# andr345/frtm-vos

Measured on AMD Instinct MI355X. Metric: segmented frames/sec/GPU (480p, ResNet101, full CG iters), higher is better.
Workload: dtype f32

## Files before the change

### frtm-vos_amd/_hip.py

```python
import ctypes
import os

import torch

_HERE = os.path.dirname(os.path.abspath(__file__))
LIB_PATH = os.path.join(_HERE, 'libfrtm_hip.so')

P, I, F, D = ctypes.c_void_p, ctypes.c_int, ctypes.c_float, ctypes.c_double


class ConvDesc(ctypes.Structure):
    _fields_ = [(k, I) for k in ('B', 'Cin', 'Hin', 'Win', 'Cout', 'ksize', 'stride', 'pad',
                                 'relu', 'out_transposed', 'splitk', 'tile', 'w_layout', 'ws_elems', 'w_pitch')]


SIGNATURES = {
    'frtm_last_error': (ctypes.c_char_p, []),
    'frtm_version': (I, []),
    'frtm_device_info': (I, [P]),
    'frtm_pixel_weights': (I, [P, I, I, I, I, F, P, P, P]),
    'frtm_normal_build': (I, [P, I, P, I, I, I, I, I, F, P, I, P, P, P, P, P]),
    'frtm_memory_next_slot': (I, [P, I, F, I, P, P, I, P]),
    'frtm_memory_insert': (I, [P, P, I, P, P]),
    'frtm_filter_scores': (I, [P, P, I, I, I, I, P, I, P]),
# ... 51 lines not shown
    'frtm_conv_persistent_launches': (ctypes.c_long, []),
    'frtm_conv_last_kernels': (ctypes.c_char_p, []),
    'frtm_conv_bf16x3_launches': (ctypes.c_long, []),
    'frtm_conv_bf16x1_launches': (ctypes.c_long, []),
    'frtm_conv_bf16x1_3x3_launches': (ctypes.c_long, []),
    'frtm_conv_bf16x1_3x3s2_launches': (ctypes.c_long, []),
    'frtm_telea_inpaint_u8': (I, [P, P, I, I, I, I, P]),
    'frtm_fastdiv_check': (ctypes.c_uint, [ctypes.c_uint, ctypes.c_uint]),
    'frtm_backbone_set_lanes': (I, [P, I]),
    'frtm_backbone_generation': (I, [P]),
    'frtm_backbone_set_winograd': (I, [P, I]),
    'frtm_backbone_set_winograd4': (I, [P, I]),
    'frtm_backbone_set_precision': (I, [P, I]),
    'frtm_backbone_set_bf16_pieces': (I, [P, I]),
    'frtm_backbone_set_bf16x1_3x3': (I, [P, I]),
    'frtm_merge_masks': (I, [P, I, I, P]),
    'frtm_merge_masks_frames': (I, [P, I, I, I, P]),
    'frtm_count_above': (I, [P, I, I, F, P, P]),
    'frtm_track_merge': (I, [P, I, I, I, P, P, P, I, P, F, P]),
    'frtm_filter_scores_pitched': (I, [P, P, I, I, I, I, P, I, I, P]),
    'frtm_bilinear_resize': (I, [P, I, I, I, P, I, I, P]),
    'frtm_tse_inject': (I, [P, P, P, P, I, I, I, I, I, I, I, P, P]),
    'frtm_cab_combine': (I, [P, P, P, I, I, I, I, I, I, I, P, P]),
    'frtm_pyrup2x': (I, [P, I, I, I, P, P]),
    'frtm_plane_mean': (I, [P, I, I, P, P]),
    'frtm_conv_wgrad_ws_elems': (ctypes.c_size_t, [I, I, I, I, I, I]),
    'frtm_conv_wgrad': (I, [P, P, I, I, I, I, I, I, P, P, P, ctypes.c_size_t, P]),
    'frtm_conv_wgrad_bf16x1_ws_elems': (ctypes.c_size_t, [I, I, I, I, I]),
    'frtm_conv_wgrad_bf16x1': (I, [P, P, I, I, I, I, I, P, P, P, ctypes.c_size_t, P]),
    'frtm_conv_wgrad_bf16x1_launches': (ctypes.c_long, []),
# ... 271 lines not shown
```

### frtm-vos_amd/build.py

```python
import os
import subprocess
import sys

HERE = os.path.dirname(os.path.abspath(__file__))
CSRC = os.path.join(HERE, 'csrc')
LIB = os.path.join(HERE, 'libfrtm_hip.so')
SOURCES = ['target_model.hip', 'target_apply_grouped.hip', 'cg_persistent.hip', 'joint_persistent.hip', 'joint_fit.hip', 'wide_maps.hip', 'conv_igemm.hip', 'conv_gemm32.hip', 'conv_wino.hip', 'conv_wino4.hip', 'conv_bf16x3.hip', 'conv_bf16x1.hip', 'conv3x3_bf16x1.hip', 'conv3x3s2_bf16x1.hip', 'conv_wgrad_bf16x1.hip', 'backbone.hip', 'image_ops.hip', 'refiner_ops.hip', 'refiner_train.hip', 'telea_host.hip', 'jf_eval.hip', 'train_step.hip', 'frame_resize.hip']
HIPCC = os.environ.get('HIPCC', '/opt/rocm/bin/hipcc')
FLAGS = ['--offload-arch=gfx950', '-O3', '-std=c++17', '-fPIC', '-Wall', '-Wno-unused-function']
if os.environ.get('FRTM_BUILD_ABLATE'):
    FLAGS.append('-DFRTM_DEBUG_ABLATE')


def _stale(target, deps):
    if not os.path.exists(target):
        return True
    t = os.path.getmtime(target)
    return any(os.path.getmtime(d) > t for d in deps)


def build(force=False, verbose=True):
    headers = [os.path.join(CSRC, 'frtm_common.h'), os.path.join(CSRC, 'conv_common.h'), os.path.join(CSRC, 'resident_grid.h'), os.path.join(CSRC, 'resample_taps.h'), os.path.join(os.path.dirname(HERE), 'include', 'frtm_hip.h'), __file__]
    objs = []
    for src in SOURCES:
        sp = os.path.join(CSRC, src)
        if not os.path.exists(sp):
            continue
        obj = os.path.join(CSRC, src.replace('.hip', '.o'))
        objs.append(obj)
        if force or _stale(obj, [sp] + headers):
            cmd = [HIPCC] + FLAGS + ['-c', sp, '-o', obj]
            if verbose:
                print(' '.join(cmd), flush=True)
            subprocess.check_call(cmd)
    if force or _stale(LIB, objs):
        cmd = [HIPCC, '--offload-arch=gfx950', '-shared', '-fPIC'] + objs + ['-o', LIB]
        if verbose:
# ... 8 lines not shown
```

### frtm-vos_amd/csrc/backbone.hip

```cpp
#include <vector>
#include <algorithm>
#include <mutex>
#include <chrono>
#include <cstdio>
#include "frtm_common.h"
#include "../../include/frtm_hip.h"

void frtm_conv_plan(int M, int Ntot, int nchunks, int vec1x1, int* tile, int* splitk);

struct ConvL {
  int Cout, Cin, ks, stride, pad;
  float* wT = nullptr; float* scale = nullptr; float* shift = nullptr; int* ktab = nullptr;
  float* wW = nullptr;
  float* wW4 = nullptr;
  float* wW6 = nullptr;
  float* wB = nullptr;
  float* wB1 = nullptr;
  float* wB3 = nullptr;
  bool loaded = false;
  int layout = 0;
  int plan_tile = 0, plan_splitk = 0;
};
struct BlockL { int conv[3]; int nconv; int ds; };

// ... 11 lines not shown
  bool bottleneck = false;
  std::vector<ConvL> convs;
  std::vector<std::vector<BlockL>> stages;
  std::vector<Lane> lanes = std::vector<Lane>(1);
  int nlanes = 1;
  hipEvent_t fork = nullptr, fork1 = nullptr;
  double last_flops = 0.0;
  double last_flops_form[4] = {0.0, 0.0, 0.0, 0.0};
  double last_flops_exec = 0.0;
  int last_launches = 0;
  bool use_winograd = true;
  int use_winograd4 = getenv("FRTM_NO_WINO4") ? 0 : getenv("FRTM_NO_WINO6") ? 1 : 2;
  int wino4_min_tiles = getenv("FRTM_WINO4_MIN_TILES") ? atoi(getenv("FRTM_WINO4_MIN_TILES")) : 256;
  int precision = 0;
  int bf16x1_min_cols = getenv("FRTM_BF16X1_MIN_COLS") ? atoi(getenv("FRTM_BF16X1_MIN_COLS")) : -1;
  bool bf16x1_3x3 = false;
  int generation = 0;
};

__global__ __launch_bounds__(256) void k_normalize_u8(const unsigned char* __restrict__ img, int H, int W, int P, const float* __restrict__ sc,
                                                       const float* __restrict__ bi, float* __restrict__ out, int planes) {
  const int Wp = W + 2 * P, Hp = H + 2 * P, q4 = (Wp + 3) / 4;
  const size_t total = (size_t)planes * Hp * q4;
  for (size_t i = (size_t)blockIdx.x * 256 + threadIdx.x; i < total; i += (size_t)gridDim.x * 256) {
    const int xq = (int)(i % q4);
    const size_t r = i / q4;
    const int yp = (int)(r % Hp), pl = (int)(r / Hp), c = pl % 3;
    const int y = yp - P;
    const float s = sc[c], b = bi[c];
    float* o = out + ((size_t)pl * Hp + yp) * Wp + xq * 4;
    const unsigned char* src = img + ((size_t)pl * H + (y < 0 || y >= H ? 0 : y)) * W;
#pragma unroll
    for (int j = 0; j < 4; ++j) {
      const int xp = xq * 4 + j, x = xp - P;
      if (xp < Wp) o[j] = (y >= 0 && y < H && x >= 0 && x < W) ? s * (float)src[x] + b : 0.f;
    }
  }
}

typedef float f32x2u __attribute__((ext_vector_type(2), aligned(4)));
__global__ __launch_bounds__(256) void k_maxpool3s2(const float* __restrict__ in, int Hin, int Win, int Ho, int Wo, float* __restrict__ out) {
  const int ox = blockIdx.x * 64 + threadIdx.x, oy = blockIdx.y * 4 + threadIdx.y;
  if (ox >= Wo || oy >= Ho) return;
  const float* ip = in + (size_t)blockIdx.z * Hin * Win;
  const int x0 = ox * 2;
  const bool left = x0 >= 1, pair = x0 + 1 < Win;
  float m = -INFINITY;
#pragma unroll
  for (int dy = 0; dy < 3; ++dy) {
    const int yy = oy * 2 - 1 + dy;
    if ((unsigned)yy >= (unsigned)Hin) continue;
    const float* row = ip + (size_t)yy * Win + x0;
// ... 145 lines not shown
  if (!c.wB3) FRTM_HIP(hipMalloc((void**)&c.wB3, FRTM_CONV_BF16X1_3X3_ELEMS(c.Cout, c.Cin) * sizeof(float)));
  const int layout = c.stride == 2 ? FRTM_WLAYOUT_BF16X1_3X3_S2 : FRTM_WLAYOUT_BF16X1_3X3;
  if (w_oihw) return frtm_conv_pack_weights(w_oihw, c.Cout, c.Cin, 3, layout, c.wB3, nullptr, (frtm_stream_t)st);
  float* tmp = nullptr;
  const size_t total = (size_t)c.Cout * c.Cin * 9;
  FRTM_HIP(hipMalloc((void**)&tmp, total * sizeof(float)));
  k_halo_to_oihw<<<(int)std::min<size_t>((total + 255) / 256, 2048), 256, 0, st>>>(c.wT, c.Cout, c.Cin, (c.Cout + 31) / 32 * 32, tmp);
  int rc = FRTM_ERR_HIP;
  if (hipGetLastError() == hipSuccess) rc = frtm_conv_pack_weights(tmp, c.Cout, c.Cin, 3, layout, c.wB3, nullptr, (frtm_stream_t)st);
  else frtm_set_error("backbone: k_halo_to_oihw failed to launch");
  (void)hipStreamSynchronize(st);
  (void)hipFree(tmp);
  return rc;
}

static int run_conv(frtm_backbone* bb, Lane& ln, int idx, int B, int Hin, int Win, const float* in, const float* residual, int relu,
                    float* out, int* Ho, int* Wo, hipStream_t st, int pad_override = -1) {
  ConvL& c = bb->convs[idx];
  if (!c.loaded) { frtm_set_error("backbone: conv %d has no weights (call frtm_backbone_set_conv)", idx); return FRTM_ERR_STATE; }
  const int pad = pad_override >= 0 ? pad_override : c.pad;
  frtm_conv_desc d;
  d.B = B; d.Cin = c.Cin; d.Hin = Hin; d.Win = Win; d.Cout = c.Cout; d.ksize = c.ks; d.stride = c.stride; d.pad = pad;
  d.relu = relu; d.out_transposed = 0; d.splitk = 0; d.tile = 0; d.w_pitch = 0; d.w_layout = c.layout; d.ws_elems = 0;
  *Ho = (Hin + 2 * pad - c.ks) / c.stride + 1;
  *Wo = (Win + 2 * pad - c.ks) / c.stride + 1;
  {
    const size_t out_elems = (size_t)c.Cout * B * (*Ho) * (*Wo);
    const size_t w = std::min((size_t)FRTM_CONV_MAX_SPLITK * out_elems, (size_t)16 * 1024 * 1024);
    int rc = ensure(bb, &ln.ws, &ln.ws_elems, std::max(w, out_elems * 2));
    if (rc) return rc;
  }
  d.ws_elems = (int)std::min<size_t>(ln.ws_elems, 0x7fffffff);
  bb->last_launches += 1;
  bb->last_flops += 2.0 * c.Cout * (double)B * (*Ho) * (*Wo) * c.Cin * c.ks * c.ks;
  if (bb->precision == 2 && bb->bf16x1_3x3 && c.wB3 && pad == 1 && !c.plan_tile && !c.plan_splitk && bf16x1_3x3_route(bb, c, B, *Ho, *Wo)) {
    d.w_layout = c.stride == 2 ? FRTM_WLAYOUT_BF16X1_3X3_S2 : FRTM_WLAYOUT_BF16X1_3X3;
    d.splitk = 1;
    bb->last_flops_exec += 2.0 * c.Cout * (double)B * (*Ho) * (*Wo) * c.Cin * 9.0;
    bb->last_flops_form[0] += 2.0 * c.Cout * (double)B * (*Ho) * (*Wo) * c.Cin * 9.0;
    return frtm_conv2d(&d, in, c.wB3, nullptr, c.scale, c.shift, residual, out, nullptr, st);
  }
  if (c.wW4 && bb->use_winograd && bb->use_winograd4) {
    int best_m = 0; long best_cost = 0, best_T = 0, best_Tp = 0;
    for (int m : {6, 4}) {
      if (m == 6 && (bb->use_winograd4 < 2 || !c.wW6)) continue;
      const int th = ceil_div(*Ho, m), tw = ceil_div(*Wo, m), NP = (m + 2) * (m + 2);
      const long T = (long)B * th * tw, Tp = (T + 63) / 64 * 64;
      if ((long)ceil_div(c.Cout, 64) * (NP * Tp / 64) < bb->wino4_min_tiles || (long)m * m * th * tw * 4 > (long)5 * (*Ho) * (*Wo) ||
          (size_t)NP * std::max(c.Cin, c.Cout) * Tp * 4 >= 0x7fffffffull)
        continue;
      if (!best_m || NP * Tp < best_cost) { best_m = m; best_cost = NP * Tp; best_T = T; best_Tp = Tp; }
    }
    if (best_m) {
      const int NP = (best_m + 2) * (best_m + 2);
      const size_t need = (size_t)NP * (c.Cin + c.Cout) * best_Tp;
      int rc = ensure(bb, &ln.ws4, &ln.ws4_elems, need);
// ... 41 lines not shown
__global__ void k_clock_probe(long long ticks, unsigned long long* out2) {
  const long long t0 = wall_clock64();
  const unsigned long long c0 = __builtin_readcyclecounter();
  long long t1 = t0;
  for (int it = 0; it < (1 << 22) && (t1 = wall_clock64()) - t0 < ticks; ++it) __builtin_amdgcn_s_sleep(32);
  out2[0] = __builtin_readcyclecounter() - c0;
  out2[1] = (unsigned long long)(t1 - t0);
}

static size_t arena_elems_per_image(const frtm_backbone* bb, int H, int W) {
  const int Hs = (H + 6 - 7) / 2 + 1, Ws = (W + 6 - 7) / 2 + 1;
  size_t need = (size_t)64 * Hs * Ws;
  int ah = (Hs + 1) / 2, aw = (Ws + 1) / 2;
  const int exp = bb->bottleneck ? 4 : 1;
  for (int s = 0; s < 4; ++s) {
    if (s > 0) { ah = (ah + 1) / 2; aw = (aw + 1) / 2; }
    need = std::max(need, (size_t)(64 << s) * exp * ah * aw);
    need = std::max(need, (size_t)(64 << s) * (s > 0 ? 4 : 1) * ah * aw);
  }
  const int P = bb->convs[0].pad;
  return std::max(need, (size_t)3 * (H + 2 * P) * (W + 2 * P));
}

static int forward_lane(frtm_backbone* bb, Lane& ln, const unsigned char* image_u8, int B, int H, int W, const float* norm_scale3,
                        const float* norm_bias3, float* layer1, float* layer2, float* layer3, float* layer4, float* layer5,
                        int stop_after_layer, hipStream_t st) {
  const size_t need = (size_t)B * arena_elems_per_image(bb, H, W);
  if (ln.buf_elems < need) {
    bb->generation += 1;
    for (auto& b : ln.buf) {
      if (b) FRTM_HIP(hipFree(b));
      b = nullptr;
      FRTM_HIP(hipMalloc((void**)&b, need * sizeof(float)));
    }
    ln.buf_elems = need;
  }
  float* norm = ln.buf[0];
  const int P = bb->convs[0].pad;
  const size_t nq = (size_t)B * 3 * (H + 2 * P) * ((W + 2 * P + 3) / 4);
  k_normalize_u8<<<(int)min((nq + 255) / 256, (size_t)8192), 256, 0, st>>>(image_u8, H, W, P, norm_scale3, norm_bias3, norm, B * 3);
  FRTM_LAUNCH_CHECK();
  int h1, w1;
  int rc = run_conv(bb, ln, 0, B, H + 2 * P, W + 2 * P, norm, nullptr, 1, ln.buf[1], &h1, &w1, st, 0);
  if (rc) return rc;
  const int Hp = (h1 + 2 - 3) / 2 + 1, Wp = (w1 + 2 - 3) / 2 + 1;
  float* x = layer1 ? layer1 : ln.buf[2];
  static const bool pool_v1 = getenv("FRTM_MAXPOOL_V1") != nullptr;
  if (pool_v1) k_maxpool3s2<<<dim3(ceil_div(Wp, 64), ceil_div(Hp, 4), B * 64), dim3(64, 4), 0, st>>>(ln.buf[1], h1, w1, Hp, Wp, x);
  else k_maxpool3s2_x4<<<dim3(ceil_div(Wp, 256), ceil_div(Hp, 4), B * 64), dim3(64, 4), 0, st>>>(ln.buf[1], h1, w1, Hp, Wp, x);
  FRTM_LAUNCH_CHECK();
  int ch = Hp, cw = Wp;
  float* taps[4] = {layer2, layer3, layer4, layer5};
  for (int s = 0; s < 4 && (s + 2) <= stop_after_layer; ++s) {
    const auto& blocks = bb->stages[s];
    for (size_t b = 0; b < blocks.size(); ++b) {
      const BlockL& bl = blocks[b];
      const bool last = (b + 1 == blocks.size());
      float* outp = (last && taps[s]) ? taps[s] : ((x == ln.buf[2]) ? ln.buf[3] : ln.buf[2]);
// ... 216 lines not shown
    if (pack) {
      FRTM_HIP(hipDeviceSynchronize());
      for (auto& c : bb->convs)
        if (wants(c)) {
          int rc = pack_bf16x1_3x3(c, nullptr, nullptr);
          if (rc) return rc;
        }
      FRTM_HIP(hipDeviceSynchronize());
    }
  }
  if ((on != 0) != bb->bf16x1_3x3) bb->generation += 1;
  bb->bf16x1_3x3 = on != 0;
  return FRTM_OK;
}

int frtm_backbone_set_winograd4(frtm_backbone_t* bb, int enable) {
  FRTM_CHECK_ARG(bb, "frtm_backbone_set_winograd4: null handle");
  bb->use_winograd4 = enable < 0 ? 0 : enable > 2 ? 2 : enable;
  return FRTM_OK;
}

static std::mutex g_lane_pool_lock;
static int lane_stream(int lane, hipStream_t* out) {
  static hipStream_t pool[16][16] = {};
  int dev = 0;
  FRTM_HIP(hipGetDevice(&dev));
  if (dev < 0 || dev >= 16 || lane < 0 || lane >= 16) { frtm_set_error("backbone: no lane stream for device %d lane %d", dev, lane); return FRTM_ERR_ARG; }
  std::lock_guard<std::mutex> hold(g_lane_pool_lock);
  if (!pool[dev][lane]) FRTM_HIP(hipStreamCreateWithFlags(&pool[dev][lane], hipStreamNonBlocking));
  *out = pool[dev][lane];
// ... 110 lines not shown
```

### frtm-vos_amd/model/feature_extractor.py

```python
import ctypes
import math
import os
from collections import OrderedDict as odict

import torch
import torch.nn as nn

from .. import _hip as H

_SPECS = {'resnet18': (18, 'basic', (2, 2, 2, 2)), 'resnet34': (34, 'basic', (3, 4, 6, 3)),
          'resnet50': (50, 'bottleneck', (3, 4, 6, 3)), 'resnet101': (101, 'bottleneck', (3, 4, 23, 3))}


class _BN(nn.Module):
    def __init__(self, c):
        super().__init__()
        self.weight = nn.Parameter(torch.ones(c), requires_grad=False)
        self.bias = nn.Parameter(torch.zeros(c), requires_grad=False)
        self.register_buffer('running_mean', torch.zeros(c))
        self.register_buffer('running_var', torch.ones(c))
        self.register_buffer('num_batches_tracked', torch.tensor(0, dtype=torch.long))
        self.eps = 1e-5


# ... 104 lines not shown
        self._handle = None
        self.device = None
        self.last_flops = 0.0
        self.last_flops_executed = 0.0
        self.last_flops_form = [0.0, 0.0, 0.0, 0.0]
        self.last_conv_launches = 0
        self.reuse_outputs = False
        self._out_cache = {}
        self._out_bufs = {}
        self._buf_serial = 0
        self.output_set = 0
        self._lanes = 1
        self._winograd = True
        self._winograd4 = not os.environ.get('FRTM_NO_WINO4')
        self._winograd6 = not os.environ.get('FRTM_NO_WINO6')
        self._precision = precision
        self.use_graph = False
        self.capture_after = 1
        self._pass_done = {}
        self.pass_frames = []
        self.pass_events = None

    @property
    def lanes(self):
        return self._lanes

    @property
    def winograd(self):
        return self._winograd

    @winograd.setter
    def winograd(self, on):
        self._winograd = bool(on)
        if self._handle is not None:
            H.call_nostream('frtm_backbone_set_winograd', self._handle, int(self._winograd))
            self._out_cache.clear()

    @property
    def winograd4(self):
        return self._winograd4

    def _wino_mode(self):
        return 0 if not self._winograd4 else 2 if self._winograd6 else 1

    @property
    def precision(self):
        return self._precision

    def _apply_precision(self, mode):
        H.call_nostream('frtm_backbone_set_bf16_pieces', self._handle, _PRECISIONS[mode])
        H.call_nostream('frtm_backbone_set_bf16x1_3x3', self._handle, int(mode == 'bf16x1_3x3'))

    @precision.setter
    def precision(self, mode):
        if mode not in _PRECISIONS:
# ... 47 lines not shown
        self.norm_bias = self.norm_bias.to(dev).contiguous()
        self.device = dev
        self.upload()
        return self

    def upload(self):
        L = H.lib()
        with torch.cuda.device(self.device):
            if self._handle is None:
                h = ctypes.c_void_p()
                H.call_nostream('frtm_backbone_create', self.arch, ctypes.byref(h))
                self._handle = h
                H.call_nostream('frtm_backbone_set_lanes', h, self._lanes)
                H.call_nostream('frtm_backbone_set_winograd', h, int(self._winograd))
                H.call_nostream('frtm_backbone_set_winograd4', h, self._wino_mode())
            pairs = self.resnet.conv_bn_pairs()
            assert L.frtm_backbone_num_convs(self._handle) == len(pairs)
            info = (ctypes.c_int * 6)()
            for i, (cv, bn) in enumerate(pairs):
                H.call_nostream('frtm_backbone_conv_info', self._handle, i, info)
                assert tuple(info[:4]) == (cv.out_channels, cv.in_channels, cv.kernel_size, cv.stride), (i, tuple(info))
                scale = (bn.weight / torch.sqrt(bn.running_var + bn.eps)).float().contiguous()
                shift = (bn.bias - bn.running_mean * scale).float().contiguous()
                H.call('frtm_backbone_set_conv', self._handle, i, H.ptr(cv.weight.data.float().contiguous()),
                       H.ptr(scale), H.ptr(shift))
            torch.cuda.current_stream().synchronize()
            self._apply_precision(self._precision)

    def lane_streams(self):
        if self._handle is None:
# ... 117 lines not shown
```

### frtm-vos_amd/ops.py

```python
import ctypes
import functools

import torch

from . import _hip as H

_workspaces = {}


def workspace(device, elems):
    if torch.cuda.is_current_stream_capturing():
        return torch.empty(int(elems), device=device, dtype=torch.float32)
    key = (device, H.stream())
    w = _workspaces.get(key)
    if w is None or w.numel() < elems:
        w = torch.empty(int(elems), device=device, dtype=torch.float32)
        _workspaces[key] = w
    return w


def padded_rows(K):
    return (K + 31) // 32 * 32


# ... 49 lines not shown
    Wo = (Win + 2 * pad - ksize) // stride + 1
    if out is None:
        out = torch.empty((B, Ho * Wo, Cout) if out_transposed else (B, Cout, Ho, Wo), device=x.device, dtype=torch.float32)
    if w_pitch > 0 and (w_pitch % 4 or wT.data_ptr() % 16):
        K, pitch = Cin * ksize * ksize, (int(w_pitch) + 3) // 4 * 4
        staged = torch.zeros(K, pitch, device=x.device, dtype=torch.float32)
        staged[:, :w_pitch].copy_(wT.reshape(-1)[:K * w_pitch].view(K, w_pitch))
        wT, w_pitch = staged, pitch
    out_elems = Cout * B * Ho * Wo
    if ws is None and splitk != 1:
        ws = workspace(x.device, min(32 * out_elems, max(2 * out_elems, 1 << 24)))
    d = H.ConvDesc(B, Cin, Hin, Win, Cout, ksize, stride, pad, int(relu), int(out_transposed), int(splitk), int(tile), int(w_layout),
                   0 if ws is None else min(ws.numel(), 0x7fffffff), int(w_pitch))
    H.call('frtm_conv2d', ctypes.byref(d), H.ptr(x), H.ptr(wT), H.ptr(ktab), H.ptr(scale), H.ptr(shift),
           H.ptr(residual), H.ptr(out), H.ptr(ws))
    return out


def filter_scores(X, f, out=None, accumulate=False, n=None, interleave=None):
    N = X.shape[0] if n is None else n
    C, h, w = X.shape[1:]
    if interleave is not None:
        batch, k, groups = interleave
        assert batch.is_contiguous() and batch.shape[0] == N * groups and tuple(batch.shape[-2:]) == (h, w)
        H.call('frtm_filter_scores_pitched', H.ptr(X), H.ptr(f), N, C, h, w, batch.data_ptr() + 4 * k * h * w, groups * h * w, int(accumulate))
        return batch
    if out is None:
        out = torch.empty(N, 1, h, w, device=X.device)
    H.call('frtm_filter_scores', H.ptr(X), H.ptr(f), N, C, h, w, H.ptr(out), int(accumulate))
    return out
# ... 451 lines not shown
```

### include/frtm_hip.h

```cpp
#ifndef FRTM_HIP_H
#define FRTM_HIP_H

#ifdef __cplusplus
extern "C" {
#endif

typedef void* frtm_stream_t;
typedef struct frtm_backbone frtm_backbone_t;

const char* frtm_last_error(void);
int frtm_version(void);
int frtm_device_info(int* out4_host);


#define FRTM_PX_PARTS 32
int frtm_pixel_weights(const void* y, int y_is_u8, int n, int H, int W, float tf,
                       float* out, float* scratch, frtm_stream_t stream);

int frtm_normal_build(const void* labels, int labels_is_u8, const float* pw, int n, int H, int W, int h, int w,
                      float tf, const int* slot_dev, int slot_host, float* Bmem, float* cmem,
                      float* scratch, const int* px_count_dev, frtm_stream_t stream);

int frtm_memory_update_window(float* sw, int cap, float lr, int num_samp_is_zero, int* state, const int* counts, int count_stride,
                              int min_count, int W, int* slots, const float* features, float* samples, int len, const float* labels,
// ... 120 lines not shown
#define FRTM_TILE_64x64 1
#define FRTM_TILE_32x64 2
#define FRTM_TILE_128x64 3
#define FRTM_TILE_64x64_8W 4
#define FRTM_TILE_64x128_8W 7
#define FRTM_TILE_128x128_8W 8
#define FRTM_TILE_128x128_16W 9
#define FRTM_TILE_80x64 10
#define FRTM_TILE_G32_64x64 23
int frtm_conv_pack_weights(const float* w_oihw, int Cout, int Cin, int ksize, int layout,
                           float* wT, int* ktab, frtm_stream_t stream);
int frtm_conv2d(const frtm_conv_desc* desc_host, const float* in, const float* wT, const int* ktab,
                const float* scale, const float* shift, const float* residual, float* out,
                float* workspace, frtm_stream_t stream);

int frtm_backbone_create(int arch, frtm_backbone_t** out_host);
int frtm_backbone_destroy(frtm_backbone_t* bb);
int frtm_backbone_num_convs(const frtm_backbone_t* bb);
int frtm_backbone_conv_info(const frtm_backbone_t* bb, int idx, int* out6_host);
int frtm_backbone_set_conv_plan(frtm_backbone_t* bb, int idx, int tile, int splitk);
int frtm_backbone_set_conv(frtm_backbone_t* bb, int idx, const float* w_oihw, const float* bn_scale,
                           const float* bn_shift, frtm_stream_t stream);
int frtm_backbone_forward(frtm_backbone_t* bb, const unsigned char* image_u8, int B, int H, int W,
                          const float* norm_scale3, const float* norm_bias3,
                          float* layer1, float* layer2, float* layer3, float* layer4, float* layer5,
                          int stop_after_layer, frtm_stream_t stream);
int frtm_backbone_forward_at(frtm_backbone_t* bb, int lane_set, const unsigned char* image_u8, int B, int H, int W, const float* norm_scale3,
                             const float* norm_bias3, float* layer1, float* layer2, float* layer3, float* layer4, float* layer5,
                             int stop_after_layer, frtm_stream_t stream);
void* frtm_backbone_lane_stream(frtm_backbone_t* bb, int lane);
// ... 6 lines not shown
long frtm_conv_bf16x1_launches(void);
long frtm_conv_bf16x1_3x3_launches(void);
long frtm_conv_bf16x1_3x3s2_launches(void);
unsigned frtm_fastdiv_check(unsigned n, unsigned d);
double frtm_backbone_last_flops(const frtm_backbone_t* bb);
double frtm_backbone_last_flops_executed(const frtm_backbone_t* bb);
double frtm_backbone_last_flops_form(const frtm_backbone_t* bb, int form);
int frtm_backbone_last_conv_launches(const frtm_backbone_t* bb);
int frtm_backbone_set_lanes(frtm_backbone_t* bb, int lanes);
int frtm_backbone_generation(const frtm_backbone_t* bb);
int frtm_backbone_set_winograd(frtm_backbone_t* bb, int enable);
int frtm_backbone_set_winograd4(frtm_backbone_t* bb, int enable);
int frtm_backbone_set_precision(frtm_backbone_t* bb, int mode);
int frtm_backbone_set_bf16_pieces(frtm_backbone_t* bb, int pieces);
int frtm_backbone_set_bf16x1_3x3(frtm_backbone_t* bb, int on);

int frtm_merge_masks(float* masks, int n_plus_1, int HW, frtm_stream_t stream);
int frtm_merge_masks_frames(float* masks, int frames, int n_plus_1, int HW, frtm_stream_t stream);
int frtm_track_merge(const float* logits, int frames, int n_obj, int HW, float* masks, unsigned char* labels, const unsigned char* lut,
                     int single_object_decode, int* counts, float thr, frtm_stream_t stream);
int frtm_filter_scores_pitched(const float* X, const float* f, int N, int C, int h, int w, float* out, int out_pitch, int accumulate,
                               frtm_stream_t stream);
int frtm_target_apply_grouped(const float* feats, size_t frame_pitch, int F, const int* frame_of_pair, const float* const* w1T,
                              const float* const* w2, int G, int Cin, int c, int h, int w, float* cft, float* scores, frtm_stream_t stream);
int frtm_count_above(const float* masks, int n, int HW, float thr, int* count, frtm_stream_t stream);

int frtm_bilinear_resize(const float* in, int planes, int h, int w, float* out, int H, int W, frtm_stream_t stream);
int frtm_tse_inject(const float* base, const float* bias, const float* ws, const float* scores, int n, int group, int C,
                    int h, int w, int H, int W, float* out, frtm_stream_t stream);
int frtm_cab_combine(const float* shallow, const float* gate, const float* deeper, int n, int C, int hd, int wd, int deeper_group,
// ... 91 lines not shown
```

Baseline: 671.8.

## Add parity-plane strided GEMM path for stride-2 backbone convolutions

Adds a new path for stride-2 convolutions (3x3, 7x7 stem, 1x1) that first splits the input into even/odd parity planes. The conv then runs as a dense implicit GEMM over contiguous plane rows, using a precomputed row-offset table. For the stem, input normalisation is fused into the plane-building kernel. Routing goes through per-shape column thresholds and skips cases where the old planner would split K. The cost is an extra plane-building pass and more workspace, and the GEMM computes some padded output columns it never uses.

```diff
diff --git a/frtm-vos_amd/_hip.py b/frtm-vos_amd/_hip.py
--- a/frtm-vos_amd/_hip.py
+++ b/frtm-vos_amd/_hip.py
@@ -89,6 +89,11 @@
     'frtm_backbone_set_precision': (I, [P, I]),
     'frtm_backbone_set_bf16_pieces': (I, [P, I]),
     'frtm_backbone_set_bf16x1_3x3': (I, [P, I]),
+    'frtm_backbone_set_strided_gemm': (I, [P, I]),
+    'frtm_conv_strided_geometry': (I, [I, I, I, I, I, I, I, P, P, I]),
+    'frtm_conv_strided_planes': (I, [P, I, I, I, I, I, I, I, P, P]),
+    'frtm_conv2d_strided': (I, [P, P, P, P, P, P, P]),
+    'frtm_conv_strided_launches': (ctypes.c_long, []),
     'frtm_merge_masks': (I, [P, I, I, P]),
     'frtm_merge_masks_frames': (I, [P, I, I, I, P]),
     'frtm_count_above': (I, [P, I, I, F, P, P]),
diff --git a/frtm-vos_amd/build.py b/frtm-vos_amd/build.py
--- a/frtm-vos_amd/build.py
+++ b/frtm-vos_amd/build.py
@@ -5,7 +5,7 @@
 HERE = os.path.dirname(os.path.abspath(__file__))
 CSRC = os.path.join(HERE, 'csrc')
 LIB = os.path.join(HERE, 'libfrtm_hip.so')
-SOURCES = ['target_model.hip', 'target_apply_grouped.hip', 'cg_persistent.hip', 'joint_persistent.hip', 'joint_fit.hip', 'wide_maps.hip', 'conv_igemm.hip', 'conv_gemm32.hip', 'conv_wino.hip', 'conv_wino4.hip', 'conv_bf16x3.hip', 'conv_bf16x1.hip', 'conv3x3_bf16x1.hip', 'conv3x3s2_bf16x1.hip', 'conv_wgrad_bf16x1.hip', 'backbone.hip', 'image_ops.hip', 'refiner_ops.hip', 'refiner_train.hip', 'telea_host.hip', 'jf_eval.hip', 'train_step.hip', 'frame_resize.hip']
+SOURCES = ['target_model.hip', 'target_apply_grouped.hip', 'cg_persistent.hip', 'joint_persistent.hip', 'joint_fit.hip', 'wide_maps.hip', 'conv_igemm.hip', 'conv_gemm32.hip', 'conv_wino.hip', 'conv_wino4.hip', 'conv_bf16x3.hip', 'conv_bf16x1.hip', 'conv3x3_bf16x1.hip', 'conv3x3s2_bf16x1.hip', 'conv_strided.hip', 'conv_wgrad_bf16x1.hip', 'backbone.hip', 'image_ops.hip', 'refiner_ops.hip', 'refiner_train.hip', 'telea_host.hip', 'jf_eval.hip', 'train_step.hip', 'frame_resize.hip']
 HIPCC = os.environ.get('HIPCC', '/opt/rocm/bin/hipcc')
 FLAGS = ['--offload-arch=gfx950', '-O3', '-std=c++17', '-fPIC', '-Wall', '-Wno-unused-function']
 if os.environ.get('FRTM_BUILD_ABLATE'):
@@ -20,7 +20,7 @@
 
 
 def build(force=False, verbose=True):
-    headers = [os.path.join(CSRC, 'frtm_common.h'), os.path.join(CSRC, 'conv_common.h'), os.path.join(CSRC, 'resident_grid.h'), os.path.join(CSRC, 'resample_taps.h'), os.path.join(os.path.dirname(HERE), 'include', 'frtm_hip.h'), __file__]
+    headers = [os.path.join(CSRC, 'frtm_common.h'), os.path.join(CSRC, 'conv_common.h'), os.path.join(CSRC, 'conv_strided.h'), os.path.join(CSRC, 'resident_grid.h'), os.path.join(CSRC, 'resample_taps.h'), os.path.join(os.path.dirname(HERE), 'include', 'frtm_hip.h'), __file__]
     objs = []
     for src in SOURCES:
         sp = os.path.join(CSRC, src)
diff --git a/frtm-vos_amd/csrc/backbone.hip b/frtm-vos_amd/csrc/backbone.hip
--- a/frtm-vos_amd/csrc/backbone.hip
+++ b/frtm-vos_amd/csrc/backbone.hip
@@ -5,6 +5,8 @@
 #include <cstdio>
 #include "frtm_common.h"
 #include "../../include/frtm_hip.h"
+
+#include "conv_strided.h"
 
 void frtm_conv_plan(int M, int Ntot, int nchunks, int vec1x1, int* tile, int* splitk);
 
@@ -49,6 +51,8 @@
   int wino4_min_tiles = getenv("FRTM_WINO4_MIN_TILES") ? atoi(getenv("FRTM_WINO4_MIN_TILES")) : 256;
   int precision = 0;
   int bf16x1_min_cols = getenv("FRTM_BF16X1_MIN_COLS") ? atoi(getenv("FRTM_BF16X1_MIN_COLS")) : -1;
+  bool strided_gemm = true;
+  int strided_min_cols = getenv("FRTM_STRIDED_MIN_COLS") ? atoi(getenv("FRTM_STRIDED_MIN_COLS")) : -1;
   bool bf16x1_3x3 = false;
   int generation = 0;
 };
@@ -71,6 +75,14 @@
       if (xp < Wp) o[j] = (y >= 0 && y < H && x >= 0 && x < W) ? s * (float)src[x] + b : 0.f;
     }
   }
+}
+
+__global__ __launch_bounds__(256) void k_normalize_u8_planes(const unsigned char* __restrict__ img, const float* __restrict__ sc, const float* __restrict__ bi,
+                                                             const PlaneParams q) {
+  parity_planes_body(q, [&](int im, int c, int y, int x) {
+    const float s = sc[c], b = bi[c];
+    return s * (float)img[((size_t)(im * 3 + c) * q.Hin + y) * q.Win + x] + b;
+  });
 }
 
 typedef float f32x2u __attribute__((ext_vector_type(2), aligned(4)));
@@ -246,6 +258,57 @@
   return rc;
 }
 
+struct StridedRule { int Cin, Cout, ks; long min_cols; };
+static const StridedRule kStridedRules[] = {
+  {128, 128, 3, 25680},
+  {256, 256, 3, 6480},
+  {512, 512, 3, 3240},
+  {3, 64, 7, 102480},
+};
+static bool old_form_splits_k(const ConvL& c, int B, int Ho, int Wo) {
+  int tile = 0, splitk = 0;
+  if (c.layout == FRTM_WLAYOUT_HALO3X3) {
+    long ptiles = -1;
+    for (int tw : {8, 16, 4}) {
+      const long w = (long)ceil_div(Ho, 64 / tw) * ceil_div(Wo, tw);
+      if (ptiles < 0 || w < ptiles) ptiles = w;
+    }
+    tile = FRTM_TILE_64x64;
+    frtm_conv_plan(c.Cout, (int)(B * ptiles * 64), ceil_div(c.Cin, 8) * 2, 0, &tile, &splitk);
+  } else {
+    frtm_conv_plan(c.Cout, B * Ho * Wo, ceil_div(c.Cin * c.ks * c.ks, 32), 0, &tile, &splitk);
+  }
+  return splitk > 1;
+}
+static bool strided_eligible(const ConvL& c) { return c.stride == 2 && ((c.ks == 3 && c.pad == 1) || (c.ks == 7 && c.pad == 3) || (c.ks == 1 && c.pad == 0)); }
+static bool strided_route(const frtm_backbone* bb, const ConvL& c, int B, int Ho, int Wo) {
+  if (!bb->strided_gemm || !strided_eligible(c) || c.plan_tile || c.plan_splitk) return false;
+  const long cols = (long)B * Ho * Wo;
+  if (bb->strided_min_cols >= 0) return cols >= bb->strided_min_cols;
+  for (const StridedRule& r : kStridedRules)
+    if (r.Cin == c.Cin && r.Cout == c.Cout && r.ks == c.ks) return cols >= r.min_cols && !old_form_splits_k(c, B, Ho, Wo);
+  return false;
+}
+
+static int run_strided(frtm_backbone* bb, Lane& ln, const ConvL& c, int B, int Hin, int Win, const float* in, int relu, float* out, int* Ho, int* Wo,
+                       hipStream_t st) {
+  const int korder = c.layout == FRTM_WLAYOUT_HALO3X3 ? 1 : 0;
+  const StridedGeom g = strided_geom(B, c.Cin, Hin, Win, c.ks, c.pad, korder);
+  if (strided_ws_elems(g) > ln.buf_elems) { frtm_set_error("backbone: the lane arena is too small for the parity planes of a %dx%d conv", c.ks, c.ks); return FRTM_ERR_STATE; }
+  *Ho = g.Ho; *Wo = g.Wo;
+  if (in) {
+    int rc = frtm_conv_strided_planes(in, B, c.Cin, Hin, Win, c.ks, c.pad, korder, ln.buf[5], (frtm_stream_t)st);
+    if (rc) return rc;
+  }
+  frtm_conv_desc d;
+  d.B = B; d.Cin = c.Cin; d.Hin = Hin; d.Win = Win; d.Cout = c.Cout; d.ksize = c.ks; d.stride = 2; d.pad = c.pad;
+  d.relu = relu; d.out_transposed = 0; d.splitk = 1; d.tile = 0; d.w_pitch = 0; d.w_layout = c.layout; d.ws_elems = 0;
+  const double flops = 2.0 * c.Cout * (double)c.Cin * c.ks * c.ks;
+  bb->last_flops_form[0] += flops * B * g.Ho * g.Wo;
+  bb->last_flops_exec += flops * g.PL;
+  return frtm_conv2d_strided(&d, ln.buf[5], c.wT, c.scale, c.shift, out, (frtm_stream_t)st);
+}
+
 static int run_conv(frtm_backbone* bb, Lane& ln, int idx, int B, int Hin, int Win, const float* in, const float* residual, int relu,
                     float* out, int* Ho, int* Wo, hipStream_t st, int pad_override = -1) {
   ConvL& c = bb->convs[idx];
@@ -272,6 +335,7 @@
     bb->last_flops_form[0] += 2.0 * c.Cout * (double)B * (*Ho) * (*Wo) * c.Cin * 9.0;
     return frtm_conv2d(&d, in, c.wB3, nullptr, c.scale, c.shift, residual, out, nullptr, st);
   }
+  if (pad == c.pad && !residual && strided_route(bb, c, B, *Ho, *Wo)) return run_strided(bb, ln, c, B, Hin, Win, in, relu, out, Ho, Wo, st);
   if (c.wW4 && bb->use_winograd && bb->use_winograd4) {
     int best_m = 0; long best_cost = 0, best_T = 0, best_Tp = 0;
     for (int m : {6, 4}) {
@@ -343,10 +407,16 @@
   int ah = (Hs + 1) / 2, aw = (Ws + 1) / 2;
   const int exp = bb->bottleneck ? 4 : 1;
   for (int s = 0; s < 4; ++s) {
-    if (s > 0) { ah = (ah + 1) / 2; aw = (aw + 1) / 2; }
+    if (s > 0) {
+      const int cin3 = bb->bottleneck ? (64 << s) : (64 << (s - 1));
+      need = std::max(need, strided_ws_elems(strided_geom(1, cin3, ah, aw, 3, 1, 1)));
+      need = std::max(need, strided_ws_elems(strided_geom(1, (64 << (s - 1)) * exp, ah, aw, 1, 0, 0)));
+      ah = (ah + 1) / 2; aw = (aw + 1) / 2;
+    }
     need = std::max(need, (size_t)(64 << s) * exp * ah * aw);
     need = std::max(need, (size_t)(64 << s) * (s > 0 ? 4 : 1) * ah * aw);
   }
+  need = std::max(need, strided_ws_elems(strided_geom(1, 3, H, W, 7, 3, 0)));
   const int P = bb->convs[0].pad;
   return std::max(need, (size_t)3 * (H + 2 * P) * (W + 2 * P));
 }
@@ -366,11 +436,22 @@
   }
   float* norm = ln.buf[0];
   const int P = bb->convs[0].pad;
-  const size_t nq = (size_t)B * 3 * (H + 2 * P) * ((W + 2 * P + 3) / 4);
-  k_normalize_u8<<<(int)min((nq + 255) / 256, (size_t)8192), 256, 0, st>>>(image_u8, H, W, P, norm_scale3, norm_bias3, norm, B * 3);
-  FRTM_LAUNCH_CHECK();
-  int h1, w1;
-  int rc = run_conv(bb, ln, 0, B, H + 2 * P, W + 2 * P, norm, nullptr, 1, ln.buf[1], &h1, &w1, st, 0);
+  int h1, w1, rc;
+  const ConvL& stem = bb->convs[0];
+  if (stem.loaded && strided_route(bb, stem, B, (H + 2 * P - stem.ks) / 2 + 1, (W + 2 * P - stem.ks) / 2 + 1)) {
+    const StridedGeom g = strided_geom(B, 3, H, W, stem.ks, P, 0);
+    const PlaneParams q = plane_params(g, ln.buf[5], (unsigned*)(ln.buf[5] + (g.s_elems + 3) / 4 * 4));
+    k_normalize_u8_planes<<<plane_grid(q), dim3(64, 4), 0, st>>>(image_u8, norm_scale3, norm_bias3, q);
+    FRTM_LAUNCH_CHECK();
+    bb->last_launches += 1;
+    bb->last_flops += 2.0 * stem.Cout * (double)B * g.Ho * g.Wo * stem.Cin * stem.ks * stem.ks;
+    rc = run_strided(bb, ln, stem, B, H, W, nullptr, 1, ln.buf[1], &h1, &w1, st);
+  } else {
+    const size_t nq = (size_t)B * 3 * (H + 2 * P) * ((W + 2 * P + 3) / 4);
+    k_normalize_u8<<<(int)min((nq + 255) / 256, (size_t)8192), 256, 0, st>>>(image_u8, H, W, P, norm_scale3, norm_bias3, norm, B * 3);
+    FRTM_LAUNCH_CHECK();
+    rc = run_conv(bb, ln, 0, B, H + 2 * P, W + 2 * P, norm, nullptr, 1, ln.buf[1], &h1, &w1, st, 0);
+  }
   if (rc) return rc;
   const int Hp = (h1 + 2 - 3) / 2 + 1, Wp = (w1 + 2 - 3) / 2 + 1;
   float* x = layer1 ? layer1 : ln.buf[2];
@@ -617,6 +698,14 @@
   return FRTM_OK;
 }
 
+int frtm_backbone_set_strided_gemm(frtm_backbone_t* bb, int on) {
+  FRTM_CHECK_ARG(bb, "frtm_backbone_set_strided_gemm: null handle");
+  FRTM_CHECK_ARG(on == 0 || on == 1, "frtm_backbone_set_strided_gemm: on must be 0 or 1, got %d", on);
+  if ((on != 0) != bb->strided_gemm) bb->generation += 1;
+  bb->strided_gemm = on != 0;
+  return FRTM_OK;
+}
+
 int frtm_backbone_set_winograd4(frtm_backbone_t* bb, int enable) {
   FRTM_CHECK_ARG(bb, "frtm_backbone_set_winograd4: null handle");
   bb->use_winograd4 = enable < 0 ? 0 : enable > 2 ? 2 : enable;
diff --git a/frtm-vos_amd/csrc/conv_strided.h b/frtm-vos_amd/csrc/conv_strided.h
--- /dev/null
+++ b/frtm-vos_amd/csrc/conv_strided.h
@@ -0,0 +1,85 @@
+#pragma once
+#include "conv_common.h"
+
+constexpr unsigned STRIDED_ZERO_ROW = 0x80000000u;
+
+struct StridedGeom {
+  int B, Cin, Hin, Win, ks, pad, korder;
+  int Ho, Wo, Hq, Wq, npl;
+  int PL;
+  int krows;
+  int slack;
+  size_t s_elems;
+};
+
+static inline StridedGeom strided_geom(int B, int Cin, int Hin, int Win, int ks, int pad, int korder) {
+  StridedGeom g;
+  g.B = B; g.Cin = Cin; g.Hin = Hin; g.Win = Win; g.ks = ks; g.pad = pad; g.korder = korder;
+  g.Ho = (Hin + 2 * pad - ks) / 2 + 1; g.Wo = (Win + 2 * pad - ks) / 2 + 1;
+  g.Hq = g.Ho + (ks - 1) / 2; g.Wq = g.Wo + (ks - 1) / 2;
+  g.npl = ks == 1 ? 1 : 4;
+  g.PL = B * g.Hq * g.Wq;
+  const int K = korder == 1 ? (Cin + 7) / 8 * 72 : Cin * ks * ks;
+  g.krows = (K + 31) / 32 * 32;
+  g.slack = ((ks - 1) / 2) * (g.Wq + 1) + 64 + 4;
+  g.s_elems = (size_t)Cin * g.npl * g.PL + g.slack;
+  return g;
+}
+static inline size_t strided_ws_elems(const StridedGeom& g) { return (g.s_elems + 3) / 4 * 4 + g.krows; }
+
+__host__ __device__ static inline unsigned strided_rowoff(int k, int Cin, int ks, int korder, int npl, int PL, int Wq) {
+  int ci, kh, kw;
+  if (korder == 1) {
+    const int ch = k / 72, r = k - ch * 72, tap = r / 8;
+    ci = ch * 8 + (r - tap * 8); kh = tap / 3; kw = tap - kh * 3;
+  } else {
+    const int kk = ks * ks;
+    ci = k / kk;
+    const int t = k - ci * kk;
+    kh = t / ks; kw = t - kh * ks;
+  }
+  if (ci >= Cin) return STRIDED_ZERO_ROW;
+  return (unsigned)((ci * npl + (npl == 1 ? 0 : (kh & 1) * 2 + (kw & 1))) * PL + (kh >> 1) * Wq + (kw >> 1)) * 4u;
+}
+
+#ifdef __HIPCC__
+struct PlaneParams {
+  int B, Cin, Hin, Win, ks, pad, korder, Hq, Wq, npl, PL, krows, slack;
+  int rows;
+  FastDiv dHq, dB;
+  float* S; unsigned* rowoff;
+};
+
+static inline PlaneParams plane_params(const StridedGeom& g, float* S, unsigned* rowoff) {
+  PlaneParams q;
+  q.B = g.B; q.Cin = g.Cin; q.Hin = g.Hin; q.Win = g.Win; q.ks = g.ks; q.pad = g.pad; q.korder = g.korder; q.Hq = g.Hq; q.Wq = g.Wq; q.npl = g.npl;
+  q.PL = g.PL; q.krows = g.krows; q.slack = g.slack;
+  q.rows = g.Cin * (g.npl == 4 ? 2 : 1) * g.B * g.Hq;
+  q.dHq = fast_div((unsigned)g.Hq); q.dB = fast_div((unsigned)g.B);
+  q.S = S; q.rowoff = rowoff;
+  return q;
+}
+static inline dim3 plane_grid(const PlaneParams& q) { return dim3((unsigned)((q.rows + 3) / 4), (unsigned)((q.Wq + 63) / 64)); }
+
+template <class Load>
+__device__ __forceinline__ void parity_planes_body(const PlaneParams& q, Load load) {
+  const int j = blockIdx.y * 64 + threadIdx.x, row = blockIdx.x * 4 + threadIdx.y;
+  if (row < q.rows && j < q.Wq) {
+    int t = fdiv(row, q.dHq);
+    const int i = row - t * q.Hq;
+    const int t2 = fdiv(t, q.dB), img = t - t2 * q.B;
+    const int a = q.npl == 4 ? (t2 & 1) : 0, ci = q.npl == 4 ? (t2 >> 1) : t2;
+    const int y = 2 * i + a - q.pad;
+    const bool yok = (unsigned)y < (unsigned)q.Hin;
+    float* dst = q.S + (size_t)(ci * q.npl + a * 2) * q.PL + (size_t)(img * q.Hq + i) * q.Wq + j;
+    const int x0 = 2 * j - q.pad;
+    dst[0] = (yok && (unsigned)x0 < (unsigned)q.Win) ? load(img, ci, y, x0) : 0.f;
+    if (q.npl == 4) dst[q.PL] = (yok && (unsigned)(x0 + 1) < (unsigned)q.Win) ? load(img, ci, y, x0 + 1) : 0.f;
+  }
+  const size_t nthreads = (size_t)gridDim.x * gridDim.y * 256;
+  const size_t gid = ((size_t)blockIdx.y * gridDim.x + blockIdx.x) * 256 + threadIdx.y * 64 + threadIdx.x;
+  float* tail = q.S + (size_t)q.Cin * q.npl * q.PL;
+  for (size_t e = gid; e < (size_t)q.slack; e += nthreads) tail[e] = 0.f;
+  for (size_t k = gid; k < (size_t)q.krows; k += nthreads) q.rowoff[k] = strided_rowoff((int)k, q.Cin, q.ks, q.korder, q.npl, q.PL, q.Wq);
+}
+#endif
diff --git a/frtm-vos_amd/csrc/conv_strided.hip b/frtm-vos_amd/csrc/conv_strided.hip
--- /dev/null
+++ b/frtm-vos_amd/csrc/conv_strided.hip
@@ -0,0 +1,216 @@
+#include <atomic>
+#include <cstdlib>
+#include <type_traits>
+#include "frtm_common.h"
+#include "../../include/frtm_hip.h"
+#include "conv_strided.h"
+
+struct StridedParams {
+  const float* S; const unsigned* rowoff; const float* wT; const float* scale; const float* shift; float* out;
+  unsigned s_bytes, w_bytes, out_bytes;
+  int M, Mp, K, nchunks;
+  int B, Ho, Wo, Hq, Wq, Ntot;
+  int relu;
+  FastDiv dMt, dHqWq, dWq;
+};
+
+__global__ __launch_bounds__(256) void k_parity_planes(const float* __restrict__ in, const PlaneParams q) {
+  const int HW = q.Hin * q.Win;
+  parity_planes_body(q, [&](int img, int ci, int y, int x) { return in[((size_t)img * q.Cin + ci) * HW + (size_t)y * q.Win + x]; });
+}
+
+__global__ __launch_bounds__(512) void k_conv_strided(const StridedParams p) {
+  constexpr int BM = 64, BN = 64, BKS = 32, LDA = BM + 16, LDB = BN + 16, LDC = BN + 4, TM = 32, TN = 16, FM = 2;
+  constexpr int STAGE = 2 * BKS * (LDA + LDB), CT = BM * LDC;
+  __shared__ __attribute__((aligned(16))) float smem[STAGE > CT ? STAGE : CT];
+  float (*As)[BKS][LDA] = reinterpret_cast<float (*)[BKS][LDA]>(smem);
+  float (*Bs)[BKS][LDB] = reinterpret_cast<float (*)[BKS][LDB]>(smem + 2 * BKS * LDA);
+
+  const int tid = threadIdx.x, lane = tid & 63, wid = tid >> 6, wm = wid >> 2, wn = wid & 3, lk = lane >> 4, li = lane & 15;
+  const int Mt = (p.M + BM - 1) / BM;
+  int m_tile, n_tile;
+  tile_order(blockIdx.x, gridDim.x, Mt, p.dMt, m_tile, n_tile);
+  const int m0 = m_tile * BM, n0 = n_tile * BN;
+  const __amdgpu_buffer_rsrc_t rin = __builtin_amdgcn_make_buffer_rsrc((void*)p.S, 0, (int)p.s_bytes, 0x00020000);
+  const __amdgpu_buffer_rsrc_t rw = __builtin_amdgcn_make_buffer_rsrc((void*)p.wT, 0, (int)p.w_bytes, 0x00020000);
+  const __amdgpu_buffer_rsrc_t rtab = __builtin_amdgcn_make_buffer_rsrc((void*)p.rowoff, 0, p.nchunks * BKS * 4, 0x00020000);
+  const __amdgpu_buffer_rsrc_t rout = __builtin_amdgcn_make_buffer_rsrc((void*)p.out, 0, (int)p.out_bytes, 0x00020000);
+
+  const int acol = (tid & 15) * 4, arow = tid >> 4;
+  const unsigned a_off = (unsigned)(m0 + acol) * 4u;
+  const unsigned a_voff = (unsigned)arow * (unsigned)(p.Mp * 4) + a_off;
+  const unsigned b_col = (unsigned)(n0 + acol) * 4u;
+  const unsigned t_voff = (unsigned)arow * 4u;
+
+  f32x4 ra, rb;
+  unsigned ro;
+  auto gload = [&](int kc) {
+    const int kb = kc * BKS;
+    rb = buf_ld4(rin, ro + b_col);
+    if (kb + BKS <= p.K) ra = buf_ld4s(rw, a_voff, (unsigned)kb * (unsigned)(p.Mp * 4));
+    else ra = buf_ld4(rw, (unsigned)(kb + arow) * (unsigned)(p.Mp * 4) + a_off);
+  };
+  auto tload = [&](int kc) { ro = __builtin_bit_cast(unsigned, buf_ld1s(rtab, t_voff, (unsigned)(kc * BKS * 4))); };
+  auto lstore = [&](int buf) {
+    *(f32x4*)&As[buf][arow][acol] = ra;
+    *(f32x4*)&Bs[buf][arow][acol] = rb;
+  };
+
+  f32x4 acc[FM];
+#pragma unroll
+  for (int i = 0; i < FM; ++i) acc[i] = f32x4{0.f, 0.f, 0.f, 0.f};
+
+  const int wu = __builtin_amdgcn_readfirstlane(wid);
+  float e_sc[8], e_sh[8];
+#pragma unroll
+  for (int e = 0; e < 8; ++e) {
+    const int mm = min(m0 + wu + e * 8, p.M - 1);
+    e_sc[e] = p.scale ? p.scale[mm] : 1.f;
+    e_sh[e] = p.scale ? p.shift[mm] : 0.f;
+  }
+  const int kc1 = p.nchunks;
+  tload(0);
+  gload(0);
+  if (kc1 > 1) tload(1);
+  lstore(0);
+  __syncthreads();
+  const unsigned a_lds = (unsigned)(size_t)(__attribute__((address_space(3))) float*)&As[0][lk][wm * TM + li];
+  const unsigned b_lds = (unsigned)(size_t)(__attribute__((address_space(3))) float*)&Bs[0][lk][wn * TN + li];
+  auto lds_rd1 = [](unsigned base, auto off) { float v; asm volatile("ds_read_b32 %0, %1 offset:%2" : "=v"(v) : "v"(base), "n"(off)); return v; };
+  auto chunk = [&](int kc, auto CUR_) {
+    constexpr int CUR = decltype(CUR_)::value;
+    const bool more = (kc + 1) < kc1;
+    if (more) { gload(kc + 1); if (kc + 2 < kc1) tload(kc + 2); }
+    float af[2][FM], bf[2];
+    constexpr int AO = CUR * BKS * LDA * 4, BO = CUR * BKS * LDB * 4;
+#pragma unroll
+    for (int i = 0; i < FM; ++i) af[0][i] = lds_rd1(a_lds, AO + i * 64);
+    bf[0] = lds_rd1(b_lds, BO);
+#pragma unroll
+    for (int kk = 0; kk < BKS / 4; ++kk) {
+      if (kk + 1 < BKS / 4) {
+#pragma unroll
+        for (int i = 0; i < FM; ++i) af[(kk + 1) & 1][i] = lds_rd1(a_lds, AO + ((kk + 1) * 4 * LDA + i * 16) * 4);
+        bf[(kk + 1) & 1] = lds_rd1(b_lds, BO + ((kk + 1) * 4 * LDB) * 4);
+        asm volatile("s_waitcnt lgkmcnt(%0)" :: "n"(FM + 1));
+      } else {
+        asm volatile("s_waitcnt lgkmcnt(0)");
+      }
+#pragma unroll
+      for (int i = 0; i < FM; ++i) asm volatile("" : "+v"(af[kk & 1][i]));
+      asm volatile("" : "+v"(bf[kk & 1]));
+#pragma unroll
+      for (int i = 0; i < FM; ++i) acc[i] = __builtin_amdgcn_mfma_f32_16x16x4f32(af[kk & 1][i], bf[kk & 1], acc[i], 0, 0, 0);
+      __builtin_amdgcn_sched_barrier(0);
+    }
+    if (more) lstore(CUR ^ 1);
+    __syncthreads();
+  };
+  {
+    int kc = 0;
+    for (; kc + 2 <= kc1; kc += 2) {
+      chunk(kc, std::integral_constant<int, 0>{});
+      chunk(kc + 1, std::integral_constant<int, 1>{});
+    }
+    if (kc < kc1) chunk(kc, std::integral_constant<int, 0>{});
+  }
+
+  float* Cs = smem;
+#pragma unroll
+  for (int i = 0; i < FM; ++i)
+#pragma unroll
+    for (int r = 0; r < 4; ++r) Cs[(wm * TM + i * 16 + lk * 4 + r) * LDC + wn * TN + li] = acc[i][r];
+  __syncthreads();
+  const int Npix = p.Ho * p.Wo, nn = n0 + lane;
+  const int img = fdiv(nn, p.dHqWq), rem = nn - img * (p.Hq * p.Wq);
+  const int ii = fdiv(rem, p.dWq), jj = rem - ii * p.Wq;
+  const unsigned o_col = (nn < p.Ntot && ii < p.Ho && jj < p.Wo) ? (unsigned)((img * p.M * Npix + ii * p.Wo + jj) * 4) : OOB;
+#pragma unroll
+  for (int e = 0; e < 8; ++e) {
+    const int row = wu + e * 8, mm = m0 + row;
+    if (mm >= p.M) break;
+    float v = Cs[row * LDC + lane];
+    if (p.scale) v = v * e_sc[e] + e_sh[e];
+    if (p.relu) v = fmaxf(v, 0.f);
+    __builtin_amdgcn_raw_buffer_store_b32(__builtin_bit_cast(unsigned, v), rout, (int)(o_col + (unsigned)(mm * Npix * 4)), 0, 0);
+  }
+}
+
+static std::atomic<long> g_strided_launches{0};
+
+static int check_geom(const char* who, int B, int Cin, int H, int W, int ks, int pad, int korder) {
+  FRTM_CHECK_ARG(B > 0 && Cin > 0 && H > 0 && W > 0 && pad >= 0, "%s: bad shape", who);
+  FRTM_CHECK_ARG(ks == 1 || ks == 3 || ks == 7, "%s: kernel size must be 1, 3 or 7 (got %d)", who, ks);
+  FRTM_CHECK_ARG(korder == 0 || (korder == 1 && ks == 3), "%s: the halo k order is for 3x3 kernels", who);
+  FRTM_CHECK_ARG(H + 2 * pad >= ks && W + 2 * pad >= ks, "%s: empty output", who);
+  return FRTM_OK;
+}
+
+extern "C" {
+
+int frtm_conv_strided_geometry(int B, int Cin, int H, int W, int ksize, int pad, int halo_order, long long* out10, int* rowoff, int rowoff_cap) {
+  int rc = check_geom("frtm_conv_strided_geometry", B, Cin, H, W, ksize, pad, halo_order);
+  if (rc) return rc;
+  FRTM_CHECK_ARG(out10, "frtm_conv_strided_geometry: null output");
+  const StridedGeom g = strided_geom(B, Cin, H, W, ksize, pad, halo_order);
+  out10[0] = g.Ho; out10[1] = g.Wo; out10[2] = g.Hq; out10[3] = g.Wq; out10[4] = g.npl; out10[5] = g.PL; out10[6] = g.krows; out10[7] = g.slack;
+  out10[8] = (long long)g.s_elems; out10[9] = (long long)strided_ws_elems(g);
+  if (rowoff) {
+    FRTM_CHECK_ARG(rowoff_cap >= g.krows, "frtm_conv_strided_geometry: the table has %d rows (room for %d)", g.krows, rowoff_cap);
+    for (int k = 0; k < g.krows; ++k) {
+      const unsigned o = strided_rowoff(k, Cin, ksize, halo_order, g.npl, g.PL, g.Wq);
+      rowoff[k] = o == STRIDED_ZERO_ROW ? -1 : (int)(o / 4);
+    }
+  }
+  return FRTM_OK;
+}
+
+int frtm_conv_strided_planes(const float* in, int B, int Cin, int H, int W, int ksize, int pad, int halo_order, float* ws, frtm_stream_t stream) {
+  conv_trace_reset();
+  int rc = check_geom("frtm_conv_strided_planes", B, Cin, H, W, ksize, pad, halo_order);
+  if (rc) return rc;
+  FRTM_CHECK_ARG(in && ws && ((size_t)ws) % 16 == 0, "frtm_conv_strided_planes: null or misaligned pointer");
+  const StridedGeom g = strided_geom(B, Cin, H, W, ksize, pad, halo_order);
+  FRTM_CHECK_ARG(strided_ws_elems(g) * 4 < 0x7fffffffull, "frtm_conv_strided_planes: planes too large for 32-bit buffer offsets");
+  const PlaneParams q = plane_params(g, ws, (unsigned*)(ws + (g.s_elems + 3) / 4 * 4));
+  k_parity_planes<<<plane_grid(q), dim3(64, 4), 0, (hipStream_t)stream>>>(in, q);
+  conv_trace("k_parity_planes");
+  FRTM_LAUNCH_CHECK();
+  return FRTM_OK;
+}
+
+int frtm_conv2d_strided(const frtm_conv_desc* d, const float* ws, const float* wT, const float* scale, const float* shift, float* out,
+                        frtm_stream_t stream) {
+  conv_trace_reset();
+  FRTM_CHECK_ARG(d && ws && wT && out, "frtm_conv2d_strided: null pointer");
+  FRTM_CHECK_ARG(d->stride == 2 && !d->out_transposed && d->w_pitch == 0 && d->splitk >= 0 && d->splitk <= 1 && d->Cout > 0,
+                 "frtm_conv2d_strided: needs stride 2, NCHW output, a packed weight image and no split-K");
+  FRTM_CHECK_ARG(d->w_layout == FRTM_WLAYOUT_GEMM || d->w_layout == FRTM_WLAYOUT_HALO3X3, "frtm_conv2d_strided: the weights are the GEMM or the halo image (layout %d)", d->w_layout);
+  FRTM_CHECK_ARG((scale == nullptr) == (shift == nullptr), "frtm_conv2d_strided: scale and shift go together");
+  const int korder = d->w_layout == FRTM_WLAYOUT_HALO3X3 ? 1 : 0;
+  int rc = check_geom("frtm_conv2d_strided", d->B, d->Cin, d->Hin, d->Win, d->ksize, d->pad, korder);
+  if (rc) return rc;
+  FRTM_CHECK_ARG(((size_t)ws) % 16 == 0 && ((size_t)wT) % 16 == 0, "frtm_conv2d_strided: planes and weights must be 16-byte aligned");
+  const StridedGeom g = strided_geom(d->B, d->Cin, d->Hin, d->Win, d->ksize, d->pad, korder);
+  StridedParams p;
+  p.S = ws; p.rowoff = (const unsigned*)(ws + (g.s_elems + 3) / 4 * 4); p.wT = wT; p.scale = scale; p.shift = shift; p.out = out;
+  p.M = d->Cout; p.Mp = (p.M + 31) / 32 * 32;
+  p.K = korder ? (d->Cin + 7) / 8 * 72 : (d->Cin * d->ksize * d->ksize + 31) / 32 * 32;
+  p.nchunks = g.krows / 32;
+  const size_t out_bytes = (size_t)d->B * p.M * g.Ho * g.Wo * 4;
+  FRTM_CHECK_ARG(g.s_elems * 4 < 0x7fffffffull && out_bytes < 0x7fffffffull && (size_t)p.K * p.Mp * 4 < 0x7fffffffull,
+                 "frtm_conv2d_strided: tensor too large for 32-bit buffer offsets");
+  p.s_bytes = (unsigned)(g.s_elems * 4); p.w_bytes = (unsigned)((size_t)p.K * p.Mp * 4); p.out_bytes = (unsigned)out_bytes;
+  p.B = d->B; p.Ho = g.Ho; p.Wo = g.Wo; p.Hq = g.Hq; p.Wq = g.Wq; p.Ntot = g.PL; p.relu = d->relu;
+  const int Mt = (p.M + 63) / 64;
+  p.dMt = fast_div((unsigned)Mt); p.dHqWq = fast_div((unsigned)(g.Hq * g.Wq)); p.dWq = fast_div((unsigned)g.Wq);
+  k_conv_strided<<<(unsigned)(Mt * ((g.PL + 63) / 64)), 512, 0, (hipStream_t)stream>>>(p);
+  g_strided_launches += 1;
+  conv_trace("k_conv_strided");
+  FRTM_LAUNCH_CHECK();
+  return FRTM_OK;
+}
+
+long frtm_conv_strided_launches(void) { return g_strided_launches.load(); }
+
+}
diff --git a/frtm-vos_amd/model/feature_extractor.py b/frtm-vos_amd/model/feature_extractor.py
--- a/frtm-vos_amd/model/feature_extractor.py
+++ b/frtm-vos_amd/model/feature_extractor.py
@@ -142,6 +142,7 @@
         self._winograd = True
         self._winograd4 = not os.environ.get('FRTM_NO_WINO4')
         self._winograd6 = not os.environ.get('FRTM_NO_WINO6')
+        self._strided_gemm = not os.environ.get('FRTM_NO_STRIDED_GEMM')
         self._precision = precision
         self.use_graph = False
         self.capture_after = 1
@@ -167,6 +168,17 @@
     @property
     def winograd4(self):
         return self._winograd4
+
+    @property
+    def strided_gemm(self):
+        return self._strided_gemm
+
+    @strided_gemm.setter
+    def strided_gemm(self, on):
+        self._strided_gemm = bool(on)
+        if self._handle is not None:
+            H.call_nostream('frtm_backbone_set_strided_gemm', self._handle, int(self._strided_gemm))
+            self._out_cache.clear()
 
     def _wino_mode(self):
         return 0 if not self._winograd4 else 2 if self._winograd6 else 1
@@ -244,6 +256,7 @@
                 H.call_nostream('frtm_backbone_set_lanes', h, self._lanes)
                 H.call_nostream('frtm_backbone_set_winograd', h, int(self._winograd))
                 H.call_nostream('frtm_backbone_set_winograd4', h, self._wino_mode())
+                H.call_nostream('frtm_backbone_set_strided_gemm', h, int(self._strided_gemm))
             pairs = self.resnet.conv_bn_pairs()
             assert L.frtm_backbone_num_convs(self._handle) == len(pairs)
             info = (ctypes.c_int * 6)()
diff --git a/frtm-vos_amd/ops.py b/frtm-vos_amd/ops.py
--- a/frtm-vos_amd/ops.py
+++ b/frtm-vos_amd/ops.py
@@ -87,6 +87,29 @@
                    0 if ws is None else min(ws.numel(), 0x7fffffff), int(w_pitch))
     H.call('frtm_conv2d', ctypes.byref(d), H.ptr(x), H.ptr(wT), H.ptr(ktab), H.ptr(scale), H.ptr(shift),
            H.ptr(residual), H.ptr(out), H.ptr(ws))
+    return out
+
+
+def strided_geometry(B, Cin, Hin, Win, ksize, pad, halo_order=False, table=False):
+    out = (ctypes.c_longlong * 10)()
+    rows = (ctypes.c_int * ((Cin + 7) // 8 * 8 * max(ksize * ksize, 9) + 64))() if table else None
+    H.call_nostream('frtm_conv_strided_geometry', B, Cin, Hin, Win, ksize, pad, int(halo_order), out, rows, 0 if rows is None else len(rows))
+    g = dict(zip(('Ho', 'Wo', 'Hq', 'Wq', 'planes', 'cols', 'krows', 'slack', 's_elems', 'ws_elems'), (int(v) for v in out)))
+    if table:
+        g['rowoff'] = list(rows[:g['krows']])
+    return g
+
+
+def conv2d_strided(x, wT, Cout, ksize, pad, w_layout=0, scale=None, shift=None, relu=False, out=None, ws=None):
+    B, Cin, Hin, Win = x.shape
+    g = strided_geometry(B, Cin, Hin, Win, ksize, pad, w_layout == 1)
+    if ws is None:
+        ws = torch.empty(g['ws_elems'], device=x.device)
+    if out is None:
+        out = torch.empty(B, Cout, g['Ho'], g['Wo'], device=x.device)
+    H.call('frtm_conv_strided_planes', H.ptr(x), B, Cin, Hin, Win, ksize, pad, int(w_layout == 1), H.ptr(ws))
+    d = H.ConvDesc(B, Cin, Hin, Win, Cout, ksize, 2, pad, int(relu), 0, 1, 0, int(w_layout), 0, 0)
+    H.call('frtm_conv2d_strided', ctypes.byref(d), H.ptr(ws), H.ptr(wT), H.ptr(scale), H.ptr(shift), H.ptr(out))
     return out
 
 
diff --git a/include/frtm_hip.h b/include/frtm_hip.h
--- a/include/frtm_hip.h
+++ b/include/frtm_hip.h
@@ -158,6 +158,12 @@
                 const float* scale, const float* shift, const float* residual, float* out,
                 float* workspace, frtm_stream_t stream);
 
+int frtm_conv_strided_geometry(int B, int Cin, int H, int W, int ksize, int pad, int halo_order, long long* out10_host, int* rowoff_host, int rowoff_cap);
+int frtm_conv_strided_planes(const float* in, int B, int Cin, int H, int W, int ksize, int pad, int halo_order, float* ws, frtm_stream_t stream);
+int frtm_conv2d_strided(const frtm_conv_desc* desc_host, const float* ws, const float* wT, const float* scale, const float* shift, float* out,
+                        frtm_stream_t stream);
+long frtm_conv_strided_launches(void);
+
 int frtm_backbone_create(int arch, frtm_backbone_t** out_host);
 int frtm_backbone_destroy(frtm_backbone_t* bb);
 int frtm_backbone_num_convs(const frtm_backbone_t* bb);
@@ -194,6 +200,7 @@
 int frtm_backbone_set_precision(frtm_backbone_t* bb, int mode);
 int frtm_backbone_set_bf16_pieces(frtm_backbone_t* bb, int pieces);
 int frtm_backbone_set_bf16x1_3x3(frtm_backbone_t* bb, int on);
+int frtm_backbone_set_strided_gemm(frtm_backbone_t* bb, int on);
 
 int frtm_merge_masks(float* masks, int n_plus_1, int HW, frtm_stream_t stream);
 int frtm_merge_masks_frames(float* masks, int frames, int n_plus_1, int HW, frtm_stream_t stream);
```

Result: no change. 669.8 (-0.3%).
